# grantjr1842/delayed-streams-modeling

Hardware: AMD Instinct MI355X
Metric: real-time stream throughput, stt-1b-en_fr @ bs=64 per GPU (Mimi encode + LM decode per 80 ms frame) (higher is better)
Workload: dtype bf16 weights + bf16 KV, f32 activations as three exact bf16 pieces, f32 accumulate (v_mfma_f32_16x16x32_bf16); 1 GPU; stt-1b-en_fr batch=64 streaming, ring KV cache full (750 frames), Mimi encode + LM decode HIP path; streams_per_gpu=64, parallelism=replicas x1 (independent stream batches, no per-step collective), streams=encoder stream || 2 LM group stream(s)

## Files before the change

delayed-streams-modeling_amd/csrc/dsm_engine_api.inc:

```

namespace {

template <typename KVT, int HD, int T>
int launch_attn_t(DsmDevice* e, hipStream_t st, float* out, const float* q, const void* k, const void* v,
                  const uint32_t* start_pos, const uint8_t* active, int B, int H, int ctx, int d, const AttnFused& fq) {
  constexpr int UNR = (sizeof(KVT) == 2 && T == 1 && HD == 128) ? 8 : 4;
  size_t lds = sizeof(float) * ((size_t)T * ctx + 4 * T * HD + 16);
  if ((long)B * H >= 2048 && (size_t)2 * ctx * HD * sizeof(KVT) >= (size_t)256 * 1024) lds += e->attn_lds_pad;
  if (lds > 64 * 1024) {
    static size_t allowed = 0;
    if (lds > allowed) {
      HIPCHK(hipFuncSetAttribute(reinterpret_cast<const void*>(&attn_kernel<KVT, HD, T, UNR>), hipFuncAttributeMaxDynamicSharedMemorySize, (int)lds));
      allowed = lds;
    }
  }
  const int tag = e->tag_attn[e->sid(st)];
  if (T == 1 && HD == 64 && ctx <= 32) {
    const int ph = e->prof_begin(tag, st);
    hipLaunchKernelGGL((attn_small_kernel<KVT, 64>), dim3((B * H + 3) / 4), dim3(256), 0, st, out, q, reinterpret_cast<const KVT*>(k),
                       reinterpret_cast<const KVT*>(v), start_pos, active, B * H, H, ctx, d, fq);
    e->prof_end(ph, st);
    HIPCHK(hipGetLastError());
    return 0;
  }
  const int ph = e->prof_begin(tag, st);
  hipLaunchKernelGGL((attn_kernel<KVT, HD, T, UNR>), dim3(B * H), dim3(256), lds, st, out, q, reinterpret_cast<const KVT*>(k),
                     reinterpret_cast<const KVT*>(v), start_pos, active, H, ctx, d, e->dev_ts_slot(tag, e->sid(st), 0), fq);
  e->prof_end(ph, st);
  HIPCHK(hipGetLastError());
  return 0;
}

template <typename KVT>
int launch_attn(DsmDevice* e, hipStream_t st, float* out, const float* q, const void* k, const void* v,
                const uint32_t* start_pos, const uint8_t* active, int B, int H, int hd, int T, int ctx, int d,
                const AttnFused& fq) {
#define DSM_ATTN(HDv, Tv) \
  if (hd == HDv && T == Tv) return launch_attn_t<KVT, HDv, Tv>(e, st, out, q, k, v, start_pos, active, B, H, ctx, d, fq);
  DSM_ATTN(32, 1) DSM_ATTN(64, 1) DSM_ATTN(128, 1) DSM_ATTN(32, 2) DSM_ATTN(64, 2) DSM_ATTN(128, 2)
#undef DSM_ATTN
  e->set_error("unsupported attention shape head_dim=%d T=%d (head_dim must be 32, 64 or 128; T 1 or 2)", hd, T);
  return DSM_ERR_INVALID;
}

int run_norm(DsmDevice* e, hipStream_t st, float* y, const float* x, const float* w, const float* b, int rows, int d,
             int rms) {
  hipLaunchKernelGGL(row_norm_kernel, dim3(rows), dim3(256), 0, st, y, x, w, b, rows, d, norm_eps(rms), rms);
  HIPCHK(hipGetLastError());
  return 0;
}

template <typename WT, typename KVT>
int transformer_layer_tail(DsmDevice* e, hipStream_t st, const TransformerW& w, int l, const ActScratch& act, int B, int T,
                           float* final_out, RowMap final_map, const float* post_norm_w, float* post_norm_out, const CaState* ca) {
  const dsm_transformer_config& c = w.cfg;
  const int d = c.d_model, H = c.num_heads, hd = d / H, M = B * T;
  const TLayerW& L = w.layers[l];
  const bool last = (l == c.num_layers - 1);
  {
    GemmArgs a = base_args(L.out_proj, act.att, plain_map(M, d), M);
    a.scale = L.ls1;
    a.res = act.x; a.rmap = plain_map(M, d);
    a.Y = act.x; a.ymap = plain_map(M, d);
    if (ca) set_norm(a, L.ncw, L.ncb, act.xn, w.ca_norm_rms);
    else set_norm(a, L.n2w, L.n2b, act.xn, c.norm);
    if (int rc = gemm_store<WT>(e, st, a)) return rc;
  }
  if (ca) {
    AttnFused none{};
    none.nt = sizeof(KVT) == 2;
    none.src = ca->src[l];
    {
      GemmArgs a = base_args(L.ca_q, act.xn, plain_map(M, d), M);
      a.Y = act.q; a.ymap = plain_map(M, d);
      Slabs sl;
      if (int rc = gemm_store<WT>(e, st, a, true, T == 1 && e->fuse_qkv ? &sl : nullptr)) return rc;
      if (sl.ws) {
        none.ws = sl.ws; none.ld = sl.ld; none.cstride = sl.cstride; none.chunks = sl.chunks;
        none.q_only = 1;
      }
    }
    if (int rc = launch_attn<KVT>(e, st, ca->att, act.q, nullptr, nullptr, ca->last, ca->act, B, H, hd, T, ca->smax, d, none)) return rc;
    GemmArgs a = base_args(L.ca_out, ca->att, plain_map(M, d), M);
    a.res = act.x; a.rmap = plain_map(M, d);
    a.Y = act.x; a.ymap = plain_map(M, d);
    set_norm(a, L.n2w, L.n2b, act.xn, c.norm);
    if (int rc = gemm_store<WT>(e, st, a)) return rc;
  }
  if (c.gating) {
    GemmArgs a = base_args(L.ff_in, act.xn, plain_map(M, d), M);
    a.N = w.hidden;
    a.nt_stride = w.hidden;
    a.Y = act.g; a.ymap = plain_map(M, w.hidden);
    if (int rc = launch_gemm<WT, KVT, EPI_GATE, 2>(e, st, a, true)) return rc;
  } else {
    GemmArgs a = base_args(L.ff_in, act.xn, plain_map(M, d), M);
    a.act = 1;
    a.Y = act.g; a.ymap = plain_map(M, w.hidden);
    if (int rc = gemm_store<WT>(e, st, a)) return rc;
  }
  GemmArgs a = base_args(L.ff_out, act.g, plain_map(M, w.hidden), M);
  a.scale = L.ls2;
  a.res = act.x; a.rmap = plain_map(M, d);
  if (last && final_out) {
    a.Y = final_out; a.ymap = final_map;
  } else {
    a.Y = act.x; a.ymap = plain_map(M, d);
  }
  if (!last) set_norm(a, w.layers[l + 1].n1w, w.layers[l + 1].n1b, act.xn, c.norm);
  else if (post_norm_out) set_norm(a, post_norm_w, nullptr, post_norm_out, c.norm);
  return gemm_store<WT>(e, st, a);
}

template <typename WT, typename KVT>
int transformer_forward(DsmDevice* e, hipStream_t st, const TransformerW& w, TransformerState& s, const ActScratch& act, int B,
                        int T, const uint8_t* d_mask, float* final_out, RowMap final_map, const float* post_norm_w = nullptr,
                        float* post_norm_out = nullptr, int phase = 0, const CaState* ca = nullptr, bool head_done = false) {
  const dsm_transformer_config& c = w.cfg;
  const int d = c.d_model, H = c.num_heads, hd = d / H, M = B * T;
  if (phase != 2 && !head_done) {
    hipLaunchKernelGGL(kv_builder_kernel, dim3(B), dim3(64), 0, st, s.pos, s.idx, d_mask, s.start_pos, s.widx,
                       c.positional_embedding == 1 ? s.rope_cs : (float*)nullptr, w.inv_freq, B, T, c.context, hd,
                       w.rope_pos_before ? 1 : 0);
    HIPCHK(hipGetLastError());
    if (int rc = run_norm(e, st, act.xn, act.x, w.layers[0].n1w, w.layers[0].n1b, M, d, c.norm)) return rc;
  }
  for (int l = 0; l < c.num_layers; ++l) {
    const TLayerW& L = w.layers[l];
    AttnFused fq{};
    fq.nt = sizeof(KVT) == 2;
    if (!(phase == 2 && l == 0)) {
      GemmArgs a = base_args(L.in_proj, act.xn, plain_map(M, d), M);
      a.Y = act.q;
      a.d = d; a.hd = hd; a.H = H; a.T = T; a.ctx = c.context;
      a.kcache = s.k[l]; a.vcache = s.v[l];
      a.widx = s.widx;
      a.rope_cs = c.positional_embedding == 1 ? s.rope_cs : nullptr;
      a.active = d_mask;
      Slabs sl;
      if (int rc = launch_gemm<WT, KVT, EPI_QKV, 1>(e, st, a, true, T == 1 && e->fuse_qkv ? &sl : nullptr)) return rc;
      if (sl.ws) {
        fq.ws = sl.ws; fq.ld = sl.ld; fq.cstride = sl.cstride; fq.chunks = sl.chunks;
        fq.rope_cs = a.rope_cs;
        fq.widx = s.widx;
      }
      if (int rc = launch_attn<KVT>(e, st, act.att, act.q, s.k[l], s.v[l], s.start_pos, d_mask, B, H, hd, T, c.context, d, fq)) return rc;
    }
    if (phase == 1) return 0;
    if (int rc = transformer_layer_tail<WT, KVT>(e, st, w, l, act, B, T, final_out, final_map, post_norm_w, post_norm_out, ca)) return rc;
  }
  return 0;
}

template <typename F>
int with_kv_type(bool kv_bf16, F&& f) {
  return kv_bf16 ? f(uint16_t{}) : f(float{});
}

int fork_groups(DsmDevice* e, hipStream_t st, size_t G) {
  if (G > 1) {
    HIPCHK(hipEventRecord(e->ev_fork, st));
    for (size_t g = 1; g < G; ++g) HIPCHK(hipStreamWaitEvent(e->s_grp[g], e->ev_fork, 0));
  }
  return 0;
}
template <typename F>
int run_groups(DsmDevice* e, hipStream_t st, size_t G, bool serialize, F&& body) {
  for (size_t g = G; g-- > 0;) {
    hipStream_t gs = (g == 0 || serialize) ? st : e->s_grp[g];
    if (int rc = body(g, gs)) return rc;
    if (g > 0) HIPCHK(hipEventRecord(e->ev_grp_done[g], gs));
  }
  return 0;
}
int join_groups(DsmDevice* e, hipStream_t st, size_t G) {
  for (size_t g = 1; g < G; ++g) HIPCHK(hipStreamWaitEvent(st, e->ev_grp_done[g], 0));
  return 0;
}

// ... 1444 lines not shown
```

delayed-streams-modeling_amd/csrc/dsm_kernels.h:

```cpp
#pragma once
#include <hip/hip_runtime.h>
#include <stdint.h>
#include "dsm_numerics.h"
#include "dsm_sampling.h"
#include "dsm_token_scores.h"
#include "dsm_text_bias.h"

typedef float f32x4 __attribute__((ext_vector_type(4)));
typedef short dsm_bf16x8 __attribute__((ext_vector_type(8)));

__device__ __forceinline__ float wave_sum64(float v) {
#pragma unroll
  for (int off = 32; off >= 1; off >>= 1) v = v + __shfl_xor(v, off, 64);
  return v;
}

enum { EPI_STORE = 0, EPI_QKV = 1, EPI_GATE = 2, EPI_RVQ = 3 };

struct RowMap {
  long bstride;
  int rpb;
  int ld;
  int toff;
  __host__ __device__ long off(int m) const { return (long)(m / rpb) * bstride + (long)((m % rpb) + toff) * ld; }
// ... 626 lines not shown
    if (EPI == EPI_GATE) {
      epi_gate(a, tot[0][mt], tot[NT - 1][mt], m, n_base + 4 * q);
    } else {
#pragma unroll
      for (int nt = 0; nt < NT; ++nt) {
        const int n = n_base + nt * a.nt_stride + 4 * q;
        if (EPI == EPI_RVQ)
          epi_rvq(a, tot[nt][mt], m, n, (n_base + nt * a.nt_stride) >> 4, q);
        else
          epi_store_qkv<KVT, EPI>(a, tot[nt][mt], m, n);
      }
    }
  }
  launch_stamp_end(a.ts);
}

template <typename KVT, int MT, int NT, int EPI, bool LOOP>
__global__ __launch_bounds__(256, 2) void gemm_bx3_kernel(GemmArgs a) {
  __shared__ __attribute__((aligned(16))) uint16_t Xp[2][3][16 * MT][32];
  launch_stamp_begin(a.ts);
  const int tid = threadIdx.x, lane = tid & 63, wave = tid >> 6;
  const int r = lane & 15, q = lane >> 4;
  const int chunks = LOOP ? 1 : (int)gridDim.y;
  const int m_base = blockIdx.z * (16 * MT);
  const int n_base = blockIdx.x * (a.wg_cols ? a.wg_cols : 64) + 16 * wave;
  const uint16_t* W = reinterpret_cast<const uint16_t*>(a.W);
  const uint16_t* wrow[NT];
#pragma unroll
  for (int nt = 0; nt < NT; ++nt) wrow[nt] = dsm_wbase<uint16_t>(a, W, n_base + nt * a.nt_stride, r, q);
  const int wst = dsm_wstep<uint16_t>(a);
  constexpr int PIECES = 16 * MT * 8;
  constexpr bool TWO = PIECES > 256;
  const bool has0 = tid < PIECES;
  const int row0 = has0 ? (tid >> 3) : 0, part = tid & 7;
  int m0 = m_base + row0;
  m0 = m0 < a.M ? m0 : a.M - 1;
  const float* xsrc0 = a.X + a.xmap.off(m0) + 4 * part;
  int m1 = m_base + row0 + 32;
  m1 = m1 < a.M ? m1 : a.M - 1;
  const float* xsrc1 = a.X + a.xmap.off(m1) + 4 * part;
  auto stage = [&](int buf, const float4& v, int row) {
    uint16_t h[4], m[4], l[4];
    dsm_split3(v.x, &h[0], &m[0], &l[0]); dsm_split3(v.y, &h[1], &m[1], &l[1]);
    dsm_split3(v.z, &h[2], &m[2], &l[2]); dsm_split3(v.w, &h[3], &m[3], &l[3]);
    const int off = row * 32 + (((part >> 1) ^ ((row >> 1) & 3)) * 8) + (part & 1) * 4;
    *reinterpret_cast<uint2*>(&Xp[buf][0][0][0] + off) = make_uint2((uint32_t)l[0] | ((uint32_t)l[1] << 16), (uint32_t)l[2] | ((uint32_t)l[3] << 16));
    *reinterpret_cast<uint2*>(&Xp[buf][1][0][0] + off) = make_uint2((uint32_t)m[0] | ((uint32_t)m[1] << 16), (uint32_t)m[2] | ((uint32_t)m[3] << 16));
    *reinterpret_cast<uint2*>(&Xp[buf][2][0][0] + off) = make_uint2((uint32_t)h[0] | ((uint32_t)h[1] << 16), (uint32_t)h[2] | ((uint32_t)h[3] << 16));
  };
  const int kb0 = LOOP ? 0 : (int)blockIdx.y * (DSM_KC >> 5);
  const int kb1 = LOOP ? (a.Kpad >> 5) : min(kb0 + (DSM_KC >> 5), a.Kpad >> 5);
  f32x4 acc[NT][MT], tot[NT][MT];
#pragma unroll
  for (int nt = 0; nt < NT; ++nt)
#pragma unroll
    for (int mt = 0; mt < MT; ++mt) {
      acc[nt][mt] = (f32x4){0.f, 0.f, 0.f, 0.f};
      tot[nt][mt] = (f32x4){0.f, 0.f, 0.f, 0.f};
    }
  float4 xa = *reinterpret_cast<const float4*>(xsrc0 + 32 * kb0);
  float4 xb = TWO ? *reinterpret_cast<const float4*>(xsrc1 + 32 * kb0) : xa;
  uint4 wv[NT];
#pragma unroll
  for (int nt = 0; nt < NT; ++nt) wv[nt] = *reinterpret_cast<const uint4*>(wrow[nt] + (long)32 * kb0 * wst);
  for (int g = kb0; g < kb1; ++g) {
    const int buf = (g - kb0) & 1;
    if (has0) stage(buf, xa, row0);
    if (TWO) stage(buf, xb, row0 + 32);
    dsm_bf16x8 wa[NT];
#pragma unroll
    for (int nt = 0; nt < NT; ++nt) {
      const uint4 w = wv[nt];
      wa[nt][0] = (short)(w.x & 0xFFFF); wa[nt][1] = (short)(w.x >> 16); wa[nt][2] = (short)(w.y & 0xFFFF); wa[nt][3] = (short)(w.y >> 16);
      wa[nt][4] = (short)(w.z & 0xFFFF); wa[nt][5] = (short)(w.z >> 16); wa[nt][6] = (short)(w.w & 0xFFFF); wa[nt][7] = (short)(w.w >> 16);
    }
    {
      const int gn = g + 1 < kb1 ? g + 1 : g;
      xa = *reinterpret_cast<const float4*>(xsrc0 + 32 * gn);
      if (TWO) xb = *reinterpret_cast<const float4*>(xsrc1 + 32 * gn);
#pragma unroll
      for (int nt = 0; nt < NT; ++nt) wv[nt] = *reinterpret_cast<const uint4*>(wrow[nt] + (long)32 * gn * wst);
    }
    __syncthreads();
#pragma unroll
    for (int p = 0; p < 3; ++p)
#pragma unroll
      for (int mt = 0; mt < MT; ++mt) {
        const int row = 16 * mt + r;
        const dsm_bf16x8 xf = *reinterpret_cast<const dsm_bf16x8*>(&Xp[buf][p][0][0] + row * 32 + ((q ^ ((row >> 1) & 3)) * 8));
#pragma unroll
        for (int nt = 0; nt < NT; ++nt) acc[nt][mt] = __builtin_amdgcn_mfma_f32_16x16x32_bf16(wa[nt], xf, acc[nt][mt], 0, 0, 0);
      }
    if (LOOP && ((g & 7) == 7 || g == kb1 - 1)) {
#pragma unroll
      for (int nt = 0; nt < NT; ++nt)
#pragma unroll
        for (int mt = 0; mt < MT; ++mt) {
          tot[nt][mt] = tot[nt][mt] + acc[nt][mt];
          acc[nt][mt] = (f32x4){0.f, 0.f, 0.f, 0.f};
        }
    }
  }
  if (!LOOP) {
#pragma unroll
    for (int nt = 0; nt < NT; ++nt)
#pragma unroll
      for (int mt = 0; mt < MT; ++mt) tot[nt][mt] = (f32x4){0.f, 0.f, 0.f, 0.f} + acc[nt][mt];
  }
  if (chunks > 1) {
    const long ld = (long)a.ws_ntiles * 16;
    const long mpad = (long)((a.M + 15) >> 4) * 16;
#pragma unroll
    for (int mt = 0; mt < MT; ++mt) {
      const int m = m_base + 16 * mt + r;
      if (m >= mpad) continue;
#pragma unroll
      for (int nt = 0; nt < NT; ++nt) {
        const int n = n_base + nt * a.nt_stride + 4 * q;
        *reinterpret_cast<f32x4*>(a.ws + ((long)blockIdx.y * mpad + m) * ld + n) = tot[nt][mt];
      }
    }
    launch_stamp_end(a.ts);
    return;
  }
#pragma unroll
  for (int mt = 0; mt < MT; ++mt) {
    const int m = m_base + 16 * mt + r;
    if (EPI == EPI_GATE) {
      epi_gate(a, tot[0][mt], tot[NT - 1][mt], m, n_base + 4 * q);
    } else {
#pragma unroll
      for (int nt = 0; nt < NT; ++nt) epi_store_qkv<KVT, EPI>(a, tot[nt][mt], m, n_base + nt * a.nt_stride + 4 * q);
    }
  }
  launch_stamp_end(a.ts);
}

__device__ __forceinline__ f32x4 slab_sum(const float* p, long cstride, int chunks) {
  f32x4 t = *reinterpret_cast<const f32x4*>(p);
  for (int c0 = 1; c0 < chunks; c0 += 8) {
    f32x4 v[8];
#pragma unroll
    for (int u = 0; u < 8; ++u) {
      const int c = c0 + u < chunks ? c0 + u : chunks - 1;
      v[u] = *reinterpret_cast<const f32x4*>(p + c * cstride);
    }
#pragma unroll
    for (int u = 0; u < 8; ++u)
      if (c0 + u < chunks) t = t + v[u];
  }
  return t;
}

template <typename KVT, int EPI>
__global__ __launch_bounds__(256) void gemm_reduce_kernel(GemmArgs a, int chunks) {
  launch_stamp_begin(a.ts ? a.ts + 2 : nullptr);
  const int lane = threadIdx.x & 63, wave = threadIdx.x >> 6;
  const int r = lane & 15, q = lane >> 4;
  const int mtiles = (a.M + 15) >> 4;
  const int out_ntiles = (a.N + 15) >> 4;
  const int t = blockIdx.x * 4 + wave;
  if (t >= mtiles * out_ntiles) return;
  const int mtile = t / out_ntiles, ntile = t % out_ntiles;
  constexpr int NT = (EPI == EPI_GATE) ? 2 : 1;
  const long ld = (long)a.ws_ntiles * 16, cstride = (long)mtiles * 16 * ld;
  const int m = mtile * 16 + r, n = ntile * 16 + 4 * q;
  f32x4 tot[NT];
#pragma unroll
  for (int nt = 0; nt < NT; ++nt) {
    tot[nt] = slab_sum(a.ws + (long)m * ld + n + nt * a.nt_stride, cstride, chunks);
  }
  if (EPI == EPI_GATE)
    epi_gate(a, tot[0], tot[NT - 1], m, n);
  else if (EPI == EPI_RVQ)
    epi_rvq(a, tot[0], m, n, ntile, q);
  else
    epi_store_qkv<KVT, EPI>(a, tot[0], m, n);
  launch_stamp_end(a.ts ? a.ts + 2 : nullptr);
}

#include "dsm_gemm_wk.h"

__device__ __forceinline__ void block_row_sums(float& s, float& s2, float* red) {
  const int lane = threadIdx.x & 63, wave = threadIdx.x >> 6;
  s = wave_sum64(s);
  s2 = wave_sum64(s2);
  if (lane == 0) { red[wave] = s; red[4 + wave] = s2; }
  __syncthreads();
  s = ((red[0] + red[1]) + red[2]) + red[3];
  s2 = ((red[4] + red[5]) + red[6]) + red[7];
}

#define DSM_ROW_ITS 4

__device__ __forceinline__ void row_norm_apply(const float4 (&v)[DSM_ROW_ITS], float s, float s2, int d, float eps, int rms,
                                               const float* __restrict__ w, const float* __restrict__ b,
                                               float* __restrict__ out) {
  float mm = 1.f, mean = 0.f, inv = 0.f;
  if (rms) {
    mm = sqrtf(s2 / (float)d + eps);
  } else {
    mean = s / (float)d;
    float var = s2 / (float)d - mean * mean;
    inv = 1.0f / sqrtf(var + eps);
  }
#pragma unroll
  for (int it = 0; it < DSM_ROW_ITS; ++it) {
    const int i = it * 1024 + 4 * (int)threadIdx.x;
    if (i < d) {
      const float4 wv = *reinterpret_cast<const float4*>(w + i);
      float4 o;
      if (rms) {
        o.x = (v[it].x / mm) * wv.x; o.y = (v[it].y / mm) * wv.y; o.z = (v[it].z / mm) * wv.z; o.w = (v[it].w / mm) * wv.w;
      } else {
        const float4 bv = *reinterpret_cast<const float4*>(b + i);
        o.x = ((v[it].x - mean) * inv) * wv.x + bv.x; o.y = ((v[it].y - mean) * inv) * wv.y + bv.y;
        o.z = ((v[it].z - mean) * inv) * wv.z + bv.z; o.w = ((v[it].w - mean) * inv) * wv.w + bv.w;
      }
      *reinterpret_cast<float4*>(out + i) = o;
    }
  }
}

template <int ITS>
__global__ __launch_bounds__(256 * ITS) void gemm_reduce_rows_kernel(GemmArgs a, int chunks) {
  constexpr int RS = ITS == 4 ? 16 : 24;
  __shared__ float red[8];
  __shared__ float carry[2][256];
  launch_stamp_begin(a.ts ? a.ts + 2 : nullptr);
  const int m = blockIdx.x;
  const int d = a.N;
  const int it = threadIdx.x >> 8, t = threadIdx.x & 255;
  const long ld = (long)a.ws_ntiles * 16, cstride = (long)((a.M + 15) >> 4) * 16 * ld;
  const int i = it * 1024 + 4 * t;
  const bool live = i < d;
  const int ic = live ? i : 0;
  const float* p = a.ws + (long)m * ld + ic;
  const f32x4 bias4 = *reinterpret_cast<const f32x4*>(a.bias ? a.bias + ic : p);
  const f32x4 scale4 = *reinterpret_cast<const f32x4*>(a.scale ? a.scale + ic : p);
  const f32x4 res4 = *reinterpret_cast<const f32x4*>(a.res ? a.res + a.rmap.off(m) + ic : p);
  const f32x4 nw4 = *reinterpret_cast<const f32x4*>(a.norm_w + ic);
  const f32x4 nb4 = *reinterpret_cast<const f32x4*>(a.norm_rms ? p : a.norm_b + ic);
  f32x4 tot = *reinterpret_cast<const f32x4*>(p);
  for (int c0 = 1; c0 < chunks; c0 += RS) {
    f32x4 w[RS];
#pragma unroll
    for (int u = 0; u < RS; ++u) {
      const int c = c0 + u < chunks ? c0 + u : chunks - 1;
      w[u] = *reinterpret_cast<const f32x4*>(p + c * cstride);
    }
    __builtin_amdgcn_sched_barrier(0);
#pragma unroll
    for (int u = 0; u < RS; ++u)
      if (c0 + u < chunks) tot = tot + w[u];
  }
  float o[4] = {tot[0], tot[1], tot[2], tot[3]};
  if (live) {
#pragma unroll
    for (int j = 0; j < 4; ++j) {
      if (a.bias) o[j] = o[j] + bias4[j];
      if (a.act == 1) o[j] = dsm_gelu_erf(o[j]);
      if (a.scale) o[j] = o[j] * scale4[j];
    }
    if (a.res) {
      o[0] = res4[0] + o[0]; o[1] = res4[1] + o[1]; o[2] = res4[2] + o[2]; o[3] = res4[3] + o[3];
    }
    *reinterpret_cast<float4*>(a.Y + a.ymap.off(m) + i) = make_float4(o[0], o[1], o[2], o[3]);
  }
  float s = 0.0f, s2 = 0.0f;
#pragma unroll
  for (int k = 0; k < ITS; ++k) {
    if (it == k) {
      if (k > 0) { s = carry[0][t]; s2 = carry[1][t]; }
      if (live) {
        s = s + o[0]; s2 = DSM_FMAF(o[0], o[0], s2);
        s = s + o[1]; s2 = DSM_FMAF(o[1], o[1], s2);
        s = s + o[2]; s2 = DSM_FMAF(o[2], o[2], s2);
        s = s + o[3]; s2 = DSM_FMAF(o[3], o[3], s2);
      }
      if (k + 1 < ITS) { carry[0][t] = s; carry[1][t] = s2; }
    }
    if (k + 1 < ITS) __syncthreads();
  }
  if (it == ITS - 1) {
    const int lane = t & 63, wave = t >> 6;
    s = wave_sum64(s);
    s2 = wave_sum64(s2);
    if (lane == 0) { red[wave] = s; red[4 + wave] = s2; }
  }
  __syncthreads();
  s = ((red[0] + red[1]) + red[2]) + red[3];
  s2 = ((red[4] + red[5]) + red[6]) + red[7];
  if (live) {
    float mm = 1.f, mean = 0.f, inv = 0.f;
    if (a.norm_rms) {
      mm = sqrtf(s2 / (float)d + a.norm_eps);
    } else {
      mean = s / (float)d;
      float var = s2 / (float)d - mean * mean;
      inv = 1.0f / sqrtf(var + a.norm_eps);
    }
    float4 r;
    if (a.norm_rms) {
      r.x = (o[0] / mm) * nw4[0]; r.y = (o[1] / mm) * nw4[1]; r.z = (o[2] / mm) * nw4[2]; r.w = (o[3] / mm) * nw4[3];
    } else {
      r.x = ((o[0] - mean) * inv) * nw4[0] + nb4[0]; r.y = ((o[1] - mean) * inv) * nw4[1] + nb4[1];
      r.z = ((o[2] - mean) * inv) * nw4[2] + nb4[2]; r.w = ((o[3] - mean) * inv) * nw4[3] + nb4[3];
    }
    *reinterpret_cast<float4*>(a.norm_out + (long)m * d + i) = r;
  }
  launch_stamp_end(a.ts ? a.ts + 2 : nullptr);
}

__global__ __launch_bounds__(256) void row_norm_kernel(float* __restrict__ y, const float* __restrict__ x,
                                                       const float* __restrict__ w, const float* __restrict__ b, int rows,
                                                       int d, float eps, int rms) {
  __shared__ float red[8];
  const int row = blockIdx.x;
  const float* xr = x + (long)row * d;
  float4 v[DSM_ROW_ITS];
  float s = 0.0f, s2 = 0.0f;
#pragma unroll
  for (int it = 0; it < DSM_ROW_ITS; ++it) {
    const int i = it * 1024 + 4 * (int)threadIdx.x;
    v[it] = make_float4(0.f, 0.f, 0.f, 0.f);
    if (i < d) {
      v[it] = *reinterpret_cast<const float4*>(xr + i);
      s = s + v[it].x; s2 = DSM_FMAF(v[it].x, v[it].x, s2);
      s = s + v[it].y; s2 = DSM_FMAF(v[it].y, v[it].y, s2);
      s = s + v[it].z; s2 = DSM_FMAF(v[it].z, v[it].z, s2);
      s = s + v[it].w; s2 = DSM_FMAF(v[it].w, v[it].w, s2);
    }
  }
  block_row_sums(s, s2, red);
  row_norm_apply(v, s, s2, d, eps, rms, w, b, y + (long)row * d);
}

struct alignas(16) AttnRowSrc {
  const void *k, *v;
};
template <typename KVT>
__device__ __forceinline__ const KVT* attn_row_base(uint64_t bits) {
  return (const KVT*)(const __attribute__((address_space(1))) KVT*)bits;
}

struct AttnFused {
  const float* ws;
  long ld, cstride;
  int chunks;
  const float* rope_cs;
  const uint32_t* widx;
  int nt;
  int q_only;
  const AttnRowSrc* src;
};

template <typename KVT, int HD, int T, int UNRB = 8>
__global__ __launch_bounds__(256, 4) void attn_kernel(float* __restrict__ out, const float* __restrict__ qbuf,
                                                   const KVT* __restrict__ kcache, const KVT* __restrict__ vcache,
                                                   const uint32_t* __restrict__ start_pos,
                                                   const uint8_t* __restrict__ active, int H, int ctx, int d,
                                                   unsigned long long* __restrict__ ts, AttnFused fq) {
  constexpr int NW = 4, LPK = HD / 8, G = 64 / LPK;
  extern __shared__ __attribute__((aligned(16))) float lds[];
  const int b = blockIdx.x / H, h = blockIdx.x % H;
  uint4 rs_kv = {0u, 0u, 0u, 0u};
  if (!kcache) {
    int bv = b;
    asm volatile("" : "+v"(bv));
    rs_kv = *reinterpret_cast<const uint4*>(fq.src + bv);
  }
  const bool ts_first = ts && threadIdx.x == 0 && blockIdx.x < 256;
  const bool ts_last = ts && threadIdx.x == 0 && blockIdx.x + 1024 >= gridDim.x;
  if (ts_first) atomicMin(&ts[0], wall_clock64());
  if (!active[b]) {
    if (ts_last) atomicMax(&ts[1], wall_clock64());
    return;
  }
  const int tid = threadIdx.x, lane = tid & 63, wave = tid >> 6;
  const int g = lane / LPK, li = lane % LPK;
  float* sc = lds;
  float* red = lds + T * ctx;
  float* scratch = red + NW * T * HD;

  const uint32_t sp = start_pos[b];
  const long e1 = (long)sp + T - 1;
  const int nvalid = (int)((e1 + 1 < (long)ctx) ? e1 + 1 : ctx);
  const float scale = (float)(1.0 / sqrt((double)HD));

  const KVT* Kb = kcache + ((long)b * H + h) * ctx * HD;
  const KVT* Vb = vcache + ((long)b * H + h) * ctx * HD;
  if (!kcache) {
    const uint64_t kp = ((uint64_t)__builtin_amdgcn_readfirstlane(rs_kv.y) << 32) | (uint32_t)__builtin_amdgcn_readfirstlane(rs_kv.x);
    const uint64_t vp = ((uint64_t)__builtin_amdgcn_readfirstlane(rs_kv.w) << 32) | (uint32_t)__builtin_amdgcn_readfirstlane(rs_kv.z);
    Kb = attn_row_base<KVT>(kp) + (long)h * ctx * HD;
    Vb = attn_row_base<KVT>(vp) + (long)h * ctx * HD;
  }
  if (T == 1 && fq.ws) {
    if (tid < (fq.q_only ? HD / 4 : 3 * HD / 4)) {
      const int part = tid / (HD / 4), i0 = 4 * (tid % (HD / 4));
      const f32x4 v = slab_sum(fq.ws + (long)b * fq.ld + part * d + h * HD + i0, fq.cstride, fq.chunks);
      float o[4] = {v[0], v[1], v[2], v[3]};
      if (part < 2 && fq.rope_cs) {
        const float4 cs = *reinterpret_cast<const float4*>(fq.rope_cs + ((long)b * (HD / 2) + (i0 >> 1)) * 2);
        const float co[2] = {cs.x, cs.z}, si[2] = {cs.y, cs.w};
#pragma unroll
        for (int p = 0; p < 2; ++p) {
          float x0 = v[2 * p], x1 = v[2 * p + 1];
          float t0 = x0 * co[p], t1 = x1 * si[p], t2 = x0 * si[p], t3 = x1 * co[p];
          o[2 * p] = t0 - t1;
          o[2 * p + 1] = t2 + t3;
        }
      }
      if (part == 0) {
        red[i0] = o[0]; red[i0 + 1] = o[1]; red[i0 + 2] = o[2]; red[i0 + 3] = o[3];
      } else {
        KVT* row = const_cast<KVT*>(part == 1 ? Kb : Vb) + (long)fq.widx[b] * HD + i0;
        store_kv4(row, o);
      }
    }
    __syncthreads();
  }
  float qv[T][8];
#pragma unroll
  for (int t = 0; t < T; ++t) {
    if (T == 1 && fq.ws) {
#pragma unroll
      for (int dd = 0; dd < 8; ++dd) qv[t][dd] = red[8 * li + dd];
    } else {
      const float* qp = qbuf + ((long)(b * T + t)) * d + h * HD + 8 * li;
      float4 q0 = *reinterpret_cast<const float4*>(qp), q1 = *reinterpret_cast<const float4*>(qp + 4);
      qv[t][0] = q0.x; qv[t][1] = q0.y; qv[t][2] = q0.z; qv[t][3] = q0.w;
      qv[t][4] = q1.x; qv[t][5] = q1.y; qv[t][6] = q1.z; qv[t][7] = q1.w;
    }
  }
  if (T == 1 && fq.ws) __syncthreads();

  constexpr int UNR = sizeof(KVT) == 2 ? UNRB : 4;
  constexpr int STEP = UNR * NW * G;
  const int jlast = nvalid - 1;
  const int last_slot = (int)(e1 % ctx);
  Raw8<KVT> ra[UNR], rb[UNR];
#define DSM_ISSUE(R, BASE, J0)                                                        \
  _Pragma("unroll") for (int u = 0; u < UNR; ++u) {                                    \
    const int jj = min((J0) + u * NW * G + g, jlast);                                  \
    if (fq.nt) R[u].load_nt(BASE + (long)jj * HD + 8 * li);                            \
    else R[u].load(BASE + (long)jj * HD + 8 * li);                                     \
  }
#define DSM_SCORES(R, J0)                                                              \
  _Pragma("unroll") for (int u = 0; u < UNR; ++u) {                                    \
    const int j = (J0) + u * NW * G + g;                                               \
    int delta = last_slot - min(j, jlast);  \
    delta += (delta < 0) ? ctx : 0;                                                    \
    float kv[8];                                                                       \
    R[u].unpack(kv);                                                                   \
    _Pragma("unroll") for (int t = 0; t < T; ++t) {                                    \
      float p = 0.0f;                                                                  \
      _Pragma("unroll") for (int dd = 0; dd < 8; ++dd) p = DSM_FMAF(qv[t][dd], kv[dd], p); \
      _Pragma("unroll") for (int off = LPK / 2; off >= 1; off >>= 1) p = p + __shfl_xor(p, off, 64); \
      if (li == 0 && j < nvalid) sc[t * ctx + j] = (delta >= T - 1 - t) ? p * scale : -DSM_INF_F; \
    }                                                                                  \
  }
  {
    int j0 = wave * G;
    DSM_ISSUE(ra, Kb, j0)
    while (j0 < nvalid) {
      DSM_ISSUE(rb, Kb, j0 + STEP)
      DSM_SCORES(ra, j0)
      j0 += STEP;
      if (j0 >= nvalid) break;
      DSM_ISSUE(ra, Kb, j0 + STEP)
      DSM_SCORES(rb, j0)
      j0 += STEP;
    }
  }
  DSM_ISSUE(ra, Vb, wave * G)
  __syncthreads();

  float lsum[T];
#pragma unroll
  for (int t = 0; t < T; ++t) {
    float m = -DSM_INF_F;
    for (int j = tid; j < nvalid; j += 256) m = fmaxf(m, sc[t * ctx + j]);
#pragma unroll
    for (int off = 32; off >= 1; off >>= 1) m = fmaxf(m, __shfl_xor(m, off, 64));
    if (lane == 0) scratch[wave] = m;
    __syncthreads();
    m = fmaxf(fmaxf(scratch[0], scratch[1]), fmaxf(scratch[2], scratch[3]));
    __syncthreads();
    float tp = 0.0f;
    for (int j = tid; j < nvalid; j += 256) {
      float p = dsm_expf(sc[t * ctx + j] - m);
      sc[t * ctx + j] = p;
      tp = tp + p;
    }
    tp = wave_sum64(tp);
    if (lane == 0) scratch[4 + wave] = tp;
    __syncthreads();
    lsum[t] = ((scratch[4] + scratch[5]) + scratch[6]) + scratch[7];
    __syncthreads();
  }

  float acc[T][8];
#pragma unroll
  for (int t = 0; t < T; ++t)
#pragma unroll
    for (int dd = 0; dd < 8; ++dd) acc[t][dd] = 0.0f;
#define DSM_PV(R, J0)                                                                  \
  _Pragma("unroll") for (int u = 0; u < UNR; ++u) {  \
    const int j = (J0) + u * NW * G + g;                                               \
    float vv[8];                                                                       \
    R[u].unpack(vv);                                                                   \
    _Pragma("unroll") for (int t = 0; t < T; ++t) {                                    \
       \
      const float wgt = (j < nvalid) ? sc[t * ctx + j] / lsum[t] : 0.0f;               \
      _Pragma("unroll") for (int dd = 0; dd < 8; ++dd) acc[t][dd] = DSM_FMAF(wgt, vv[dd], acc[t][dd]); \
    }                                                                                  \
  }
  {
    int j0 = wave * G;
    while (j0 < nvalid) {
      DSM_ISSUE(rb, Vb, j0 + STEP)
      DSM_PV(ra, j0)
      j0 += STEP;
      if (j0 >= nvalid) break;
      DSM_ISSUE(ra, Vb, j0 + STEP)
      DSM_PV(rb, j0)
      j0 += STEP;
    }
  }
#undef DSM_ISSUE
#undef DSM_SCORES
#undef DSM_PV
#pragma unroll
  for (int t = 0; t < T; ++t)
#pragma unroll
    for (int dd = 0; dd < 8; ++dd) {
      float v = acc[t][dd];
#pragma unroll
      for (int off = 32; off >= LPK; off >>= 1) v = v + __shfl_xor(v, off, 64);
      acc[t][dd] = v;
    }
  if (g == 0) {
#pragma unroll
    for (int t = 0; t < T; ++t)
#pragma unroll
      for (int dd = 0; dd < 8; ++dd) red[(wave * T + t) * HD + 8 * li + dd] = acc[t][dd];
  }
  __syncthreads();
  for (int i = tid; i < T * HD; i += 256) {
    int t = i / HD, dd = i % HD;
    float tot = ((red[(0 * T + t) * HD + dd] + red[(1 * T + t) * HD + dd]) + red[(2 * T + t) * HD + dd]) +
                red[(3 * T + t) * HD + dd];
    out[((long)(b * T + t)) * d + h * HD + dd] = tot;
  }
  if (ts_last) atomicMax(&ts[1], wall_clock64());
}

template <typename KVT, int HD>
__global__ __launch_bounds__(256) void attn_small_kernel(float* __restrict__ out, const float* __restrict__ qbuf,
                                                         const KVT* __restrict__ kcache, const KVT* __restrict__ vcache,
                                                         const uint32_t* __restrict__ start_pos, const uint8_t* __restrict__ active,
                                                         int BH, int H, int ctx, int d, AttnFused fq) {
  static_assert(HD == 64, "one lane group of 8 lanes per key");
  constexpr int LPK = HD / 8;
  __shared__ __attribute__((aligned(16))) float lds_all[4][32 + HD];
  const int tid = threadIdx.x, lane = tid & 63, wave = tid >> 6;
  const int unit = blockIdx.x * 4 + wave;
  const int uc = unit < BH ? unit : BH - 1;
  const int b = uc / H, h = uc % H;
  const bool on = unit < BH && active[b];
  float* sc = lds_all[wave];
  float* qs = sc + 32;
  const int g = lane / LPK, li = lane % LPK;
  const uint32_t sp = start_pos[b];
  const long e1 = (long)sp;
  const int nvalid = (int)((e1 + 1 < (long)ctx) ? e1 + 1 : ctx);
  const float scale = (float)(1.0 / sqrt((double)HD));
  const KVT* Kb = kcache + ((long)b * H + h) * ctx * HD;
  const KVT* Vb = vcache + ((long)b * H + h) * ctx * HD;
  if (!kcache) {
    Kb = attn_row_base<KVT>((uint64_t)fq.src[b].k) + (long)h * ctx * HD;
    Vb = attn_row_base<KVT>((uint64_t)fq.src[b].v) + (long)h * ctx * HD;
  }
  if (fq.ws) {
    if (on && lane < (fq.q_only ? HD / 4 : 3 * HD / 4)) {
      const int part = lane / (HD / 4), i0 = 4 * (lane % (HD / 4));
      const f32x4 v = slab_sum(fq.ws + (long)b * fq.ld + part * d + h * HD + i0, fq.cstride, fq.chunks);
      float o[4] = {v[0], v[1], v[2], v[3]};
      if (part < 2 && fq.rope_cs) {
        const float4 cs = *reinterpret_cast<const float4*>(fq.rope_cs + ((long)b * (HD / 2) + (i0 >> 1)) * 2);
        const float co[2] = {cs.x, cs.z}, si[2] = {cs.y, cs.w};
#pragma unroll
        for (int p = 0; p < 2; ++p) {
          float x0 = v[2 * p], x1 = v[2 * p + 1];
          float t0 = x0 * co[p], t1 = x1 * si[p], t2 = x0 * si[p], t3 = x1 * co[p];
          o[2 * p] = t0 - t1;
          o[2 * p + 1] = t2 + t3;
        }
      }
      if (part == 0) {
        qs[i0] = o[0]; qs[i0 + 1] = o[1]; qs[i0 + 2] = o[2]; qs[i0 + 3] = o[3];
      } else {
        KVT* row = const_cast<KVT*>(part == 1 ? Kb : Vb) + (long)fq.widx[b] * HD + i0;
        store_kv4(row, o);
      }
    }
    __syncthreads();
  }
  if (!on) return;
  float qv[8];
  if (fq.ws) {
#pragma unroll
    for (int dd = 0; dd < 8; ++dd) qv[dd] = qs[8 * li + dd];
  } else {
    const float* qp = qbuf + (long)b * d + h * HD + 8 * li;
    const float4 q0 = *reinterpret_cast<const float4*>(qp), q1 = *reinterpret_cast<const float4*>(qp + 4);
    qv[0] = q0.x; qv[1] = q0.y; qv[2] = q0.z; qv[3] = q0.w; qv[4] = q1.x; qv[5] = q1.y; qv[6] = q1.z; qv[7] = q1.w;
  }
  const int jlast = nvalid - 1;
  Raw8<KVT> rk[4], rv[4];
#pragma unroll
  for (int w = 0; w < 4; ++w) {
    const int jj = min(8 * w + g, jlast);
    rk[w].load(Kb + (long)jj * HD + 8 * li);
  }
#pragma unroll
  for (int w = 0; w < 4; ++w) {
    const int jj = min(8 * w + g, jlast);
    rv[w].load(Vb + (long)jj * HD + 8 * li);
  }
#pragma unroll
  for (int w = 0; w < 4; ++w) {
    const int j = 8 * w + g;
    float kv[8];
    rk[w].unpack(kv);
    float p = 0.0f;
#pragma unroll
    for (int dd = 0; dd < 8; ++dd) p = DSM_FMAF(qv[dd], kv[dd], p);
#pragma unroll
    for (int off = LPK / 2; off >= 1; off >>= 1) p = p + __shfl_xor(p, off, 64);
    if (li == 0 && j < nvalid) sc[j] = p * scale;
  }
  float m = -DSM_INF_F;
  if (lane < nvalid) m = fmaxf(m, sc[lane]);
#pragma unroll
  for (int off = 32; off >= 1; off >>= 1) m = fmaxf(m, __shfl_xor(m, off, 64));
  float tp = 0.0f;
  if (lane < nvalid) {
    const float p = dsm_expf(sc[lane] - m);
    sc[lane] = p;
    tp = tp + p;
  }
  tp = wave_sum64(tp);
  const float lsum = ((tp + 0.0f) + 0.0f) + 0.0f;
  float tot[8];
#pragma unroll
  for (int w = 0; w < 4; ++w) {
    const int j = 8 * w + g;
    float vv[8];
    rv[w].unpack(vv);
    const float wgt = (j < nvalid) ? sc[j] / lsum : 0.0f;
#pragma unroll
    for (int dd = 0; dd < 8; ++dd) {
      float v = (j < nvalid) ? DSM_FMAF(wgt, vv[dd], 0.0f) : 0.0f;
#pragma unroll
      for (int off = 32; off >= LPK; off >>= 1) v = v + __shfl_xor(v, off, 64);
      tot[dd] = w == 0 ? v : tot[dd] + v;
    }
  }
  if (g == 0) {
    float* o = out + (long)b * d + h * HD + 8 * li;
    *reinterpret_cast<float4*>(o) = make_float4(tot[0], tot[1], tot[2], tot[3]);
    *reinterpret_cast<float4*>(o + 4) = make_float4(tot[4], tot[5], tot[6], tot[7]);
  }
}

__global__ void kv_builder_kernel(uint32_t* __restrict__ pos, uint32_t* __restrict__ idx,
                                  const uint8_t* __restrict__ active, uint32_t* __restrict__ start_pos,
                                  uint32_t* __restrict__ widx, float* __restrict__ rope_cs,
                                  const float* __restrict__ inv_freq, int B, int T, int ctx, int hd,
                                  int rope_before) {
  const int b = blockIdx.x;
  if (b >= B) return;
  __shared__ uint32_t s_pos_after;
  if (threadIdx.x == 0) {
    uint32_t p = pos[b], i = idx[b];
    const uint32_t p0 = p;
    start_pos[b] = p;
    for (int t = 0; t < T; ++t) widx[b * T + t] = active[b] ? (uint32_t)((i + t) % ctx) : i;
    if (active[b]) {
      pos[b] = p + T;
      idx[b] = (uint32_t)((i + T) % ctx);
      p += T;
    }
    s_pos_after = rope_before ? p0 : p;
  }
  __syncthreads();
  if (rope_cs) {
    const int half = hd / 2;
    for (int e = threadIdx.x; e < T * half; e += blockDim.x) {
      int t = e / half, i = e % half;
      float ang = (float)(s_pos_after + (uint32_t)t) * inv_freq[i];
      float s, c;
      dsm_sincosf(ang, &s, &c);
      rope_cs[((long)(b * T + t) * half + i) * 2] = c;
      rope_cs[((long)(b * T + t) * half + i) * 2 + 1] = s;
    }
  }
}
// ... 1349 lines not shown
```

Baseline: 1853 x realtime (stream-seconds of audio per wall second).

## Issue K-cache and QKV slab loads early in fused decode attention kernel

Splits the attention kernel into a templated body with two variants. The fused T=1 variant issues the first K-tile loads and the QKV split-K slab loads before the active check and the Q/K/V reduction, so that memory latency overlaps the prologue. If the freshly written K row falls inside the first prefetched tile, that row is reloaded. The PV loop now double-buffers V by issuing both ra and rb up front, and the softmax weights are normalised once in LDS instead of being divided per key in the PV loop. In exchange, register pressure rises and inactive blocks now do speculative loads.

```diff
diff --git a/delayed-streams-modeling_amd/csrc/dsm_engine_api.inc b/delayed-streams-modeling_amd/csrc/dsm_engine_api.inc
--- a/delayed-streams-modeling_amd/csrc/dsm_engine_api.inc
+++ b/delayed-streams-modeling_amd/csrc/dsm_engine_api.inc
@@ -7,11 +7,16 @@
   constexpr int UNR = (sizeof(KVT) == 2 && T == 1 && HD == 128) ? 8 : 4;
   size_t lds = sizeof(float) * ((size_t)T * ctx + 4 * T * HD + 16);
   if ((long)B * H >= 2048 && (size_t)2 * ctx * HD * sizeof(KVT) >= (size_t)256 * 1024) lds += e->attn_lds_pad;
+  auto kernel = &attn_plain_kernel<KVT, HD, T, UNR>;
+  if constexpr (T == 1) {
+    if (fq.ws && k) kernel = &attn_kernel<KVT, HD, T, UNR>;
+  }
   if (lds > 64 * 1024) {
-    static size_t allowed = 0;
-    if (lds > allowed) {
-      HIPCHK(hipFuncSetAttribute(reinterpret_cast<const void*>(&attn_kernel<KVT, HD, T, UNR>), hipFuncAttributeMaxDynamicSharedMemorySize, (int)lds));
-      allowed = lds;
+    static size_t allowed[2] = {0, 0};
+    size_t& a = allowed[kernel != &attn_plain_kernel<KVT, HD, T, UNR>];
+    if (lds > a) {
+      HIPCHK(hipFuncSetAttribute(reinterpret_cast<const void*>(kernel), hipFuncAttributeMaxDynamicSharedMemorySize, (int)lds));
+      a = lds;
     }
   }
   const int tag = e->tag_attn[e->sid(st)];
@@ -24,7 +29,7 @@
     return 0;
   }
   const int ph = e->prof_begin(tag, st);
-  hipLaunchKernelGGL((attn_kernel<KVT, HD, T, UNR>), dim3(B * H), dim3(256), lds, st, out, q, reinterpret_cast<const KVT*>(k),
+  hipLaunchKernelGGL(kernel, dim3(B * H), dim3(256), lds, st, out, q, reinterpret_cast<const KVT*>(k),
                      reinterpret_cast<const KVT*>(v), start_pos, active, H, ctx, d, e->dev_ts_slot(tag, e->sid(st), 0), fq);
   e->prof_end(ph, st);
   HIPCHK(hipGetLastError());
diff --git a/delayed-streams-modeling_amd/csrc/dsm_kernels.h b/delayed-streams-modeling_amd/csrc/dsm_kernels.h
--- a/delayed-streams-modeling_amd/csrc/dsm_kernels.h
+++ b/delayed-streams-modeling_amd/csrc/dsm_kernels.h
@@ -802,6 +802,37 @@
   return t;
 }
 
+__device__ __forceinline__ void slab_issue(const float* p, long cstride, int chunks, f32x4& s0, f32x4 (&s8)[8]) {
+  s0 = *reinterpret_cast<const f32x4*>(p);
+  if (chunks > 1) {
+#pragma unroll
+    for (int u = 0; u < 8; ++u) {
+      const int c = 1 + u < chunks ? 1 + u : chunks - 1;
+      s8[u] = *reinterpret_cast<const f32x4*>(p + c * cstride);
+    }
+  }
+}
+__device__ __forceinline__ f32x4 slab_finish(const float* p, long cstride, int chunks, const f32x4& s0, const f32x4 (&s8)[8]) {
+  f32x4 t = s0;
+  if (chunks > 1) {
+#pragma unroll
+    for (int u = 0; u < 8; ++u)
+      if (1 + u < chunks) t = t + s8[u];
+  }
+  for (int c0 = 9; c0 < chunks; c0 += 8) {
+    f32x4 v[8];
+#pragma unroll
+    for (int u = 0; u < 8; ++u) {
+      const int c = c0 + u < chunks ? c0 + u : chunks - 1;
+      v[u] = *reinterpret_cast<const f32x4*>(p + c * cstride);
+    }
+#pragma unroll
+    for (int u = 0; u < 8; ++u)
+      if (c0 + u < chunks) t = t + v[u];
+  }
+  return t;
+}
+
 template <typename KVT, int EPI>
 __global__ __launch_bounds__(256) void gemm_reduce_kernel(GemmArgs a, int chunks) {
   launch_stamp_begin(a.ts ? a.ts + 2 : nullptr);
@@ -1005,54 +1036,81 @@
   const AttnRowSrc* src;
 };
 
-template <typename KVT, int HD, int T, int UNRB = 8>
-__global__ __launch_bounds__(256, 4) void attn_kernel(float* __restrict__ out, const float* __restrict__ qbuf,
-                                                   const KVT* __restrict__ kcache, const KVT* __restrict__ vcache,
-                                                   const uint32_t* __restrict__ start_pos,
-                                                   const uint8_t* __restrict__ active, int H, int ctx, int d,
-                                                   unsigned long long* __restrict__ ts, AttnFused fq) {
+template <typename KVT, int HD, int T, int UNRB, bool EARLY>
+__device__ __forceinline__ void attn_body(float* __restrict__ out, const float* __restrict__ qbuf,
+                                          const KVT* __restrict__ kcache, const KVT* __restrict__ vcache,
+                                          const uint32_t* __restrict__ start_pos,
+                                          const uint8_t* __restrict__ active, int H, int ctx, int d,
+                                          unsigned long long* __restrict__ ts, const AttnFused& fq) {
+  static_assert(!EARLY || T == 1, "the fused prologue is T = 1 only");
   constexpr int NW = 4, LPK = HD / 8, G = 64 / LPK;
   extern __shared__ __attribute__((aligned(16))) float lds[];
   const int b = blockIdx.x / H, h = blockIdx.x % H;
+  const bool fused = EARLY || (T == 1 && fq.ws);
+  const uint8_t* actp = active + b;
+  const unsigned actsh = (unsigned)(reinterpret_cast<uintptr_t>(actp) & 3);
+  const uint32_t actw = *reinterpret_cast<const uint32_t*>(actp - actsh);
+  const uint32_t sp = start_pos[b];
+  const uint32_t wi = *(fused && !fq.q_only ? fq.widx + b : start_pos + b);
+  const bool ts_first = ts && threadIdx.x == 0 && blockIdx.x < 256;
+  const bool ts_last = ts && threadIdx.x == 0 && blockIdx.x + 1024 >= gridDim.x;
+  if (ts_first) atomicMin(&ts[0], wall_clock64());
+  const int tid = threadIdx.x, lane = tid & 63, wave = tid >> 6;
+  const int g = lane / LPK, li = lane % LPK;
+  constexpr int UNR = sizeof(KVT) == 2 ? UNRB : 4;
+  constexpr int STEP = UNR * NW * G;
+  Raw8<KVT> ra[UNR], rb[UNR];
+  const int nslab = fq.q_only ? HD / 4 : 3 * HD / 4;
+  const int part = tid / (HD / 4), i0 = 4 * (tid % (HD / 4));
+  const bool roped = part < 2 && fq.rope_cs;
+  float* sc = lds;
+  float* red = lds + T * ctx;
+  float* scratch = red + NW * T * HD;
+  const float* slab = fq.ws + (long)b * fq.ld + part * d + h * HD + i0;
+  f32x4 s0, s8[8];
+  float4 cs;
   uint4 rs_kv = {0u, 0u, 0u, 0u};
-  if (!kcache) {
+  if (!EARLY && !kcache) {
     int bv = b;
     asm volatile("" : "+v"(bv));
     rs_kv = *reinterpret_cast<const uint4*>(fq.src + bv);
   }
-  const bool ts_first = ts && threadIdx.x == 0 && blockIdx.x < 256;
-  const bool ts_last = ts && threadIdx.x == 0 && blockIdx.x + 1024 >= gridDim.x;
-  if (ts_first) atomicMin(&ts[0], wall_clock64());
-  if (!active[b]) {
+  if constexpr (EARLY) {
+    if (tid < nslab) {
+      slab_issue(slab, fq.cstride, fq.chunks, s0, s8);
+      if (roped) cs = *reinterpret_cast<const float4*>(fq.rope_cs + ((long)b * (HD / 2) + (i0 >> 1)) * 2);
+    }
+    const KVT* K0 = kcache + ((long)b * H + h) * ctx * HD + 8 * li;
+    int jj[UNR];
+#pragma unroll
+    for (int u = 0; u < UNR; ++u) jj[u] = min(wave * G + u * NW * G + g, ctx - 1);
+#pragma unroll
+    for (int u = 0; u < UNR; ++u) {
+      if (fq.nt) ra[u].load_nt(K0 + (long)jj[u] * HD);
+      else ra[u].load(K0 + (long)jj[u] * HD);
+    }
+  }
+  if (!((actw >> (8 * actsh)) & 0xFFu)) {
     if (ts_last) atomicMax(&ts[1], wall_clock64());
     return;
   }
-  const int tid = threadIdx.x, lane = tid & 63, wave = tid >> 6;
-  const int g = lane / LPK, li = lane % LPK;
-  float* sc = lds;
-  float* red = lds + T * ctx;
-  float* scratch = red + NW * T * HD;
-
-  const uint32_t sp = start_pos[b];
-  const long e1 = (long)sp + T - 1;
-  const int nvalid = (int)((e1 + 1 < (long)ctx) ? e1 + 1 : ctx);
-  const float scale = (float)(1.0 / sqrt((double)HD));
-
   const KVT* Kb = kcache + ((long)b * H + h) * ctx * HD;
   const KVT* Vb = vcache + ((long)b * H + h) * ctx * HD;
-  if (!kcache) {
+  if (!EARLY && !kcache) {
     const uint64_t kp = ((uint64_t)__builtin_amdgcn_readfirstlane(rs_kv.y) << 32) | (uint32_t)__builtin_amdgcn_readfirstlane(rs_kv.x);
     const uint64_t vp = ((uint64_t)__builtin_amdgcn_readfirstlane(rs_kv.w) << 32) | (uint32_t)__builtin_amdgcn_readfirstlane(rs_kv.z);
     Kb = attn_row_base<KVT>(kp) + (long)h * ctx * HD;
     Vb = attn_row_base<KVT>(vp) + (long)h * ctx * HD;
   }
-  if (T == 1 && fq.ws) {
-    if (tid < (fq.q_only ? HD / 4 : 3 * HD / 4)) {
-      const int part = tid / (HD / 4), i0 = 4 * (tid % (HD / 4));
-      const f32x4 v = slab_sum(fq.ws + (long)b * fq.ld + part * d + h * HD + i0, fq.cstride, fq.chunks);
+  if (fused) {
+    if (tid < nslab) {
+      if constexpr (!EARLY) {
+        slab_issue(slab, fq.cstride, fq.chunks, s0, s8);
+        if (roped) cs = *reinterpret_cast<const float4*>(fq.rope_cs + ((long)b * (HD / 2) + (i0 >> 1)) * 2);
+      }
+      const f32x4 v = slab_finish(slab, fq.cstride, fq.chunks, s0, s8);
       float o[4] = {v[0], v[1], v[2], v[3]};
-      if (part < 2 && fq.rope_cs) {
-        const float4 cs = *reinterpret_cast<const float4*>(fq.rope_cs + ((long)b * (HD / 2) + (i0 >> 1)) * 2);
+      if (roped) {
         const float co[2] = {cs.x, cs.z}, si[2] = {cs.y, cs.w};
 #pragma unroll
         for (int p = 0; p < 2; ++p) {
@@ -1065,16 +1123,28 @@
       if (part == 0) {
         red[i0] = o[0]; red[i0 + 1] = o[1]; red[i0 + 2] = o[2]; red[i0 + 3] = o[3];
       } else {
-        KVT* row = const_cast<KVT*>(part == 1 ? Kb : Vb) + (long)fq.widx[b] * HD + i0;
+        KVT* row = const_cast<KVT*>(part == 1 ? Kb : Vb) + (long)wi * HD + i0;
         store_kv4(row, o);
       }
     }
     __syncthreads();
-  }
+    if (EARLY && !fq.q_only && wi < (uint32_t)STEP && (int)(wi / G) % NW == wave) {
+#pragma unroll
+      for (int u = 0; u < UNR; ++u) {
+        if ((int)wi == wave * G + u * NW * G + g) {
+          if (fq.nt) ra[u].load_nt(Kb + (long)wi * HD + 8 * li);
+          else ra[u].load(Kb + (long)wi * HD + 8 * li);
+        }
+      }
+    }
+  }
+  const long e1 = (long)sp + T - 1;
+  const int nvalid = (int)((e1 + 1 < (long)ctx) ? e1 + 1 : ctx);
+  const float scale = (float)(1.0 / sqrt((double)HD));
   float qv[T][8];
 #pragma unroll
   for (int t = 0; t < T; ++t) {
-    if (T == 1 && fq.ws) {
+    if (fused) {
 #pragma unroll
       for (int dd = 0; dd < 8; ++dd) qv[t][dd] = red[8 * li + dd];
     } else {
@@ -1084,13 +1154,10 @@
       qv[t][4] = q1.x; qv[t][5] = q1.y; qv[t][6] = q1.z; qv[t][7] = q1.w;
     }
   }
-  if (T == 1 && fq.ws) __syncthreads();
-
-  constexpr int UNR = sizeof(KVT) == 2 ? UNRB : 4;
-  constexpr int STEP = UNR * NW * G;
+  if (fused) __syncthreads();
+
   const int jlast = nvalid - 1;
   const int last_slot = (int)(e1 % ctx);
-  Raw8<KVT> ra[UNR], rb[UNR];
 #define DSM_ISSUE(R, BASE, J0)                                                        \
   _Pragma("unroll") for (int u = 0; u < UNR; ++u) {                                    \
     const int jj = min((J0) + u * NW * G + g, jlast);                                  \
@@ -1113,7 +1180,7 @@
   }
   {
     int j0 = wave * G;
-    DSM_ISSUE(ra, Kb, j0)
+    if (!EARLY) DSM_ISSUE(ra, Kb, j0)
     while (j0 < nvalid) {
       DSM_ISSUE(rb, Kb, j0 + STEP)
       DSM_SCORES(ra, j0)
@@ -1125,6 +1192,7 @@
     }
   }
   DSM_ISSUE(ra, Vb, wave * G)
+  DSM_ISSUE(rb, Vb, wave * G + STEP)
   __syncthreads();
 
   float lsum[T];
@@ -1148,6 +1216,7 @@
     if (lane == 0) scratch[4 + wave] = tp;
     __syncthreads();
     lsum[t] = ((scratch[4] + scratch[5]) + scratch[6]) + scratch[7];
+    for (int j = tid; j < nvalid; j += 256) sc[t * ctx + j] = sc[t * ctx + j] / lsum[t];
     __syncthreads();
   }
 
@@ -1163,20 +1232,21 @@
     R[u].unpack(vv);                                                                   \
     _Pragma("unroll") for (int t = 0; t < T; ++t) {                                    \
        \
-      const float wgt = (j < nvalid) ? sc[t * ctx + j] / lsum[t] : 0.0f;               \
+      const float wgt = (j < nvalid) ? sc[t * ctx + j] : 0.0f;                         \
       _Pragma("unroll") for (int dd = 0; dd < 8; ++dd) acc[t][dd] = DSM_FMAF(wgt, vv[dd], acc[t][dd]); \
     }                                                                                  \
   }
   {
     int j0 = wave * G;
     while (j0 < nvalid) {
-      DSM_ISSUE(rb, Vb, j0 + STEP)
       DSM_PV(ra, j0)
       j0 += STEP;
       if (j0 >= nvalid) break;
       DSM_ISSUE(ra, Vb, j0 + STEP)
       DSM_PV(rb, j0)
       j0 += STEP;
+      if (j0 >= nvalid) break;
+      DSM_ISSUE(rb, Vb, j0 + STEP)
     }
   }
 #undef DSM_ISSUE
@@ -1206,6 +1276,20 @@
   }
   if (ts_last) atomicMax(&ts[1], wall_clock64());
 }
+
+#define DSM_ATTN_PARAMS                                                                                                   \
+  float *__restrict__ out, const float *__restrict__ qbuf, const KVT *__restrict__ kcache, const KVT *__restrict__ vcache, \
+      const uint32_t *__restrict__ start_pos, const uint8_t *__restrict__ active, int H, int ctx, int d,                  \
+      unsigned long long *__restrict__ ts, AttnFused fq
+template <typename KVT, int HD, int T, int UNRB = 8>
+__global__ __launch_bounds__(256, 4) void attn_kernel(DSM_ATTN_PARAMS) {
+  attn_body<KVT, HD, T, UNRB, true>(out, qbuf, kcache, vcache, start_pos, active, H, ctx, d, ts, fq);
+}
+template <typename KVT, int HD, int T, int UNRB = 8>
+__global__ __launch_bounds__(256, 4) void attn_plain_kernel(DSM_ATTN_PARAMS) {
+  attn_body<KVT, HD, T, UNRB, false>(out, qbuf, kcache, vcache, start_pos, active, H, ctx, d, ts, fq);
+}
+#undef DSM_ATTN_PARAMS
 
 template <typename KVT, int HD>
 __global__ __launch_bounds__(256) void attn_small_kernel(float* __restrict__ out, const float* __restrict__ qbuf,
```

Result: no change. 1863 x realtime (stream-seconds of audio per wall second) (median of 6 runs) (+0.5%).
